# JiangongChen/ORB_SLAM3-1

Measured on AMD Instinct MI355X. Metric: tracking frames/s (ORB extract+match), higher is better.
Workload: dtype u8; 1 GPU; ORBextractor 640x480, 8 levels, 1000 features (configs[1]) + SearchByBoW 1000x1000 per frame (configs[2]); batch_per_gpu=256

## Files before the change

include/orbslam3_hip.h:

```cpp
#ifndef ORBSLAM3_HIP_H
#define ORBSLAM3_HIP_H

#include <stddef.h>
#include <stdint.h>

#ifdef __cplusplus
extern "C" {
#endif

#define ORBX_OK 0
#define ORBX_ERR_EMPTY (-1)
#define ORBX_ERR_CAPACITY (-2)
#define ORBX_ERR_ARG (-3)
#define ORBX_ERR_NO_DEVICE (-4)
#define ORBX_ERR_HIP (-5)
#define ORBX_ERR_INTERNAL (-6)

const char* orbx_last_error(void);
int orbx_device_count(void);


typedef struct OrbxKeyPoint {
    float x, y;
    float size;
// ... 36 lines not shown
                        const OrbxKeyPoint* kps_r, const uint8_t* desc_r, int n_r, float mb, float mbf, float* u_right, float* depth);
int orbx_stereo_matches_device(orbx_extractor* left, orbx_extractor* right, int batch,
                               const OrbxKeyPoint* d_kps_l, const uint8_t* d_desc_l, const int32_t* d_n_l,
                               const OrbxKeyPoint* d_kps_r, const uint8_t* d_desc_r, const int32_t* d_n_r, int cap,
                               float mb, float mbf, float* d_u_right, float* d_depth, void* stream);

int orbx_profile_enable(orbx_extractor* h, int on);
int orbx_profile_read(orbx_extractor* h, float* stage_ms, int n_stages);

int orbx_debug_blurred_level(orbx_extractor* h, int frame, int level, uint8_t* dst, int dst_stride);
int orbx_debug_candidates(orbx_extractor* h, int frame, int level, OrbxKeyPoint* out, int cap, int* n);
int orbx_debug_level_keypoints(orbx_extractor* h, int frame, int level, OrbxKeyPoint* out, int cap, int* n);
int orbx_debug_set_fast_corner_cap(orbx_extractor* h, int cap);
int orbx_debug_set_tail_delay(orbx_extractor* h, int microseconds);
int orbx_debug_last_schedule(orbx_extractor* h);
int orbx_debug_octree_waves(orbx_extractor* h, int launch);
int orbx_debug_octree_table(orbx_extractor* h, int level, int* depth, int* n_ini, int16_t* bounds, int cap);
int orbx_debug_resize_bands(orbx_extractor* h);
int orbx_debug_resize_rows(int src_h, int dst_h, uint32_t* rows, int* band_rows);
int orbx_debug_fast_scores(const uint8_t* patches, int n, int pitch, int* out);
int orbx_debug_orient_desc(orbx_extractor* h, int width, int height, int batch, const uint8_t* raw, const uint8_t* blurred, int pad_byte,
                           const int32_t* counts, const int32_t* keys, int cap, int guard_rows,
                           OrbxKeyPoint* kps, uint8_t* desc, OrbxKeyPoint* lvl_kps, int lvl_cap, int32_t* sel_caps);


int orbm_hamming(const uint8_t a[32], const uint8_t b[32]);

typedef struct OrbmFeatVec {
    int32_t n_nodes;
    const uint32_t* node_id;
// ... 514 lines not shown
```

orb_slam3-1_amd/capi.py:

```python
import ctypes as C
import os

import numpy as np

_PKG_DIR = os.path.dirname(os.path.abspath(__file__))
_LIB_PATH = os.path.join(_PKG_DIR, "liborbslam3_hip.so")

KP_DTYPE = np.dtype([("x", "f4"), ("y", "f4"), ("size", "f4"), ("angle", "f4"), ("response", "f4"),
                     ("octave", "i4"), ("class_id", "i4")])
assert KP_DTYPE.itemsize == 28

ORBX_OK, ORBX_ERR_EMPTY, ORBX_ERR_CAPACITY, ORBX_ERR_ARG, ORBX_ERR_NO_DEVICE, ORBX_ERR_HIP, ORBX_ERR_INTERNAL = 0, -1, -2, -3, -4, -5, -6


class OrbxError(RuntimeError):
    def __init__(self, code, msg):
        super().__init__("orbslam3_hip error %d: %s" % (code, msg))
        self.code = code


class FeatVec(C.Structure):
    _fields_ = [("n_nodes", C.c_int32), ("node_id", C.c_void_p), ("offset", C.c_void_p), ("feat", C.c_void_p)]


# ... 44 lines not shown
                                          C.c_void_p, C.c_void_p, C.c_int, C.c_void_p, C.c_void_p, C.c_void_p, C.c_void_p]
lib.orbx_max_keypoints.argtypes = [C.c_void_p]
lib.orbx_max_keypoints_for.argtypes = [C.c_void_p, C.c_int, C.c_int]
lib.orbx_levels.argtypes = [C.c_void_p]
lib.orbx_scale_factor.argtypes = [C.c_void_p]
lib.orbx_scale_factor.restype = C.c_float
lib.orbx_scale_tables.argtypes = [C.c_void_p] + [C.c_void_p] * 4
lib.orbx_features_per_level.argtypes = [C.c_void_p, C.c_void_p]
lib.orbx_pyramid_level_size.argtypes = [C.c_void_p, C.c_int, C.POINTER(C.c_int), C.POINTER(C.c_int)]
lib.orbx_pyramid_level.argtypes = [C.c_void_p, C.c_int, C.c_int, C.c_int, C.c_void_p, C.c_int]
lib.orbx_debug_blurred_level.argtypes = [C.c_void_p, C.c_int, C.c_int, C.c_void_p, C.c_int]
lib.orbx_debug_candidates.argtypes = [C.c_void_p, C.c_int, C.c_int, C.c_void_p, C.c_int, C.POINTER(C.c_int)]
lib.orbx_debug_level_keypoints.argtypes = [C.c_void_p, C.c_int, C.c_int, C.c_void_p, C.c_int, C.POINTER(C.c_int)]
lib.orbx_debug_set_tail_delay.argtypes = [C.c_void_p, C.c_int]
lib.orbx_debug_last_schedule.argtypes = [C.c_void_p]
lib.orbx_debug_octree_waves.argtypes = [C.c_void_p, C.c_int]
lib.orbx_debug_octree_table.argtypes = [C.c_void_p, C.c_int, C.POINTER(C.c_int), C.POINTER(C.c_int), C.c_void_p, C.c_int]
lib.orbx_debug_resize_bands.argtypes = [C.c_void_p]
lib.orbx_debug_resize_rows.argtypes = [C.c_int, C.c_int, C.c_void_p, C.POINTER(C.c_int)]
lib.orbx_debug_introsort.argtypes = [C.c_void_p, C.c_void_p, C.c_void_p, C.c_int]
lib.orbx_debug_wave_sort.argtypes = [C.c_void_p, C.c_void_p, C.c_void_p, C.c_int]
lib.orbx_debug_fast_scores.argtypes = [C.c_void_p, C.c_int, C.c_int, C.c_void_p]
lib.orbx_debug_orient_desc.argtypes = [C.c_void_p, C.c_int, C.c_int, C.c_int, C.c_void_p, C.c_void_p, C.c_int, C.c_void_p, C.c_void_p,
                                       C.c_int, C.c_int, C.c_void_p, C.c_void_p, C.c_void_p, C.c_int, C.c_void_p]
lib.orbx_debug_fast_atan2.restype = C.c_float
lib.orbx_debug_fast_atan2.argtypes = [C.c_float, C.c_float]
lib.orbx_debug_sincos.argtypes = [C.c_float, C.POINTER(C.c_float), C.POINTER(C.c_float)]


def _p(a):
# ... 138 lines not shown
        _check(lib.orbx_debug_blurred_level(self._h, frame, level, _p(out), out.strides[0]))
        return out

    def debug_set_fast_corner_cap(self, cap):
        lib.orbx_debug_set_fast_corner_cap.argtypes = [C.c_void_p, C.c_int]
        _check(lib.orbx_debug_set_fast_corner_cap(self._h, int(cap)))

    def debug_set_tail_delay(self, microseconds):
        _check(lib.orbx_debug_set_tail_delay(self._h, int(microseconds)))

    def debug_resize_bands(self):
        return bool(lib.orbx_debug_resize_bands(self._h))

    def debug_last_schedule(self):
        return int(lib.orbx_debug_last_schedule(self._h))

    def debug_octree_waves(self, launch):
        return int(lib.orbx_debug_octree_waves(self._h, launch))

    def debug_octree_table(self, level):
        depth, n_ini = C.c_int(), C.c_int()
        out = np.zeros(2 * 65537, np.int16)
        n = _check(lib.orbx_debug_octree_table(self._h, level, C.byref(depth), C.byref(n_ini), _p(out), out.size))
        nb = (1 << depth.value) + 1
        assert n == (n_ini.value + 1) * nb or n == 0
        return depth.value, n_ini.value, out[:n_ini.value * nb].reshape(n_ini.value, nb).copy(), out[n_ini.value * nb:n].copy()

    def candidates(self, level, frame=0, cap=200000):
        out = np.zeros(cap, KP_DTYPE)
        n = C.c_int()
# ... 2259 lines not shown
```

orb_slam3-1_amd/csrc/orbx_extractor.hip:

```cpp
#include <hip/hip_runtime.h>

#include <algorithm>
#include <cmath>
#include <cstdarg>
#include <cstdio>
#include <cstdlib>
#include <cstring>
#include <string>
#include <vector>

#include "hip_check.h"
#include "orbx_kernels.hip"

namespace orbx {

thread_local std::string g_last_error;

int fail(int code, const char* fmt, ...)
{
    char buf[512];
    va_list ap;
    va_start(ap, fmt);
    vsnprintf(buf, sizeof(buf), fmt, ap);
    va_end(ap);
// ... 65 lines not shown
        if (count <= n) return ORBX_OK;
        if (p) { (void)hipFree(p); p = nullptr; n = 0; }
        ORBX_HIP(hipMalloc((void**)&p, count * sizeof(T)));
        n = count;
        return ORBX_OK;
    }
    int upload(const std::vector<T>& v)
    {
        int r = ensure(v.size() ? v.size() : 1);
        if (r) return r;
        if (!v.empty()) ORBX_HIP(hipMemcpy(p, v.data(), v.size() * sizeof(T), hipMemcpyHostToDevice));
        return ORBX_OK;
    }
    void release() { if (p) (void)hipFree(p); p = nullptr; n = 0; }
};

}

using namespace orbx;

struct orbx_extractor {
    int device = 0;
    int nfeatures = 0, nlevels = 0, ini_th = 0, min_th = 0;
    float scale_factor_f = 0;
    double scale_factor_d = 0;
    std::vector<float> scale, inv_scale, sigma2, inv_sigma2;
    std::vector<int> nfeat;
    int taps[7];
    int max_kp = 0;

// ... 65 lines not shown
    int oct_split = 0, oct_pool_hi = 0;
    size_t oct_lds_hi = 0;
    int split_parts = 1;
    bool serial_schedule = false;
    bool last_resize_bands = false;
    int resize_band_min = 64;
    int resize_tail_first = 4;
    bool oct_dyn_off = false;
    int oct_dyn_max_batch = 64;
    int oct_waves_env = 0;
    int oct_waves_beside[3] = {2, 2, 2};
    int oct_small_max_waves = 32;
    int last_oct_waves[3] = {0, 0, 0};
    int oct_dyn_keys_beside = 6144;
    bool resize_beside = true;
    std::vector<hipStream_t> aux_streams;
    hipEvent_t ev_parts_fork = nullptr;
    std::vector<hipEvent_t> ev_parts_join;

    int setup_geometry(int w, int h);
    int ensure_batch(int batch);
    int enqueue(const uint8_t* d_imgs, bool level0_ready, int batch, int row_stride, size_t frame_stride,
                int lap0, int lap1, OrbxKeyPoint* o_kps, uint8_t* o_desc, int cap, int* o_n, int* o_mono, int* o_status,
                hipStream_t st);
    int launch_orient_desc(int f0, int n_frames, hipStream_t s, OrbxKeyPoint* o_kps, uint8_t* o_desc, int cap);
};

static void build_tables(orbx_extractor* e)
{
    const int nl = e->nlevels;
// ... 116 lines not shown
            while (c1 < (int)cells.size() && cells[c1].y0 == cells[c0].y0) c1++;
            const int n_row = c1 - c0;
            const int w_cell = std::max(cells[c0].x1 - cells[c0].x0 - 6, 1);
            static const int strip_width = getenv("ORBX_STRIP_WIDTH") ? std::max(48, std::min(atoi(getenv("ORBX_STRIP_WIDTH")), 250)) : kStripWidth;
            const int per = std::max(1, std::min(kStripMaxCells, (strip_width - 6) / w_cell));
            const int n_strips_row = (n_row + per - 1) / per;
            for (int k = 0; k < n_strips_row; k++) {
                const int a = c0 + (int)((long long)n_row * k / n_strips_row), b = c0 + (int)((long long)n_row * (k + 1) / n_strips_row);
                StripDesc sd;
                sd.level = (int16_t)l; sd.cell0 = (int16_t)a; sd.ncell = (int16_t)(b - a);
                sd.x0 = cells[a].x0; sd.x1 = cells[b - 1].x1; sd.y0 = cells[a].y0; sd.y1 = cells[a].y1; sd.pad = 0;
                strips.push_back(sd);
            }
            c0 = c1;
        }
        for (int y0 = 0; y0 < L.h; y0 += kBlurTH)
            for (int x0 = 0; x0 < L.w; x0 += kBlurTW) {
                TileDesc t; t.level = (int16_t)l; t.x0 = (int16_t)x0; t.y0 = (int16_t)y0;
                t.edge = (int16_t)((x0 == 0 ? 1 : 0) | (L.w <= x0 + kBlurTW + 2 ? 2 : 0));
                tiles.push_back(t);
            }
        if (l > 0) {
            const LevelDesc& P = levels[l - 1];
            const double scale_x = 1. / ((double)L.w / P.w);
            const int wpad = round_up(L.w, 4);
            std::vector<int> xofs(wpad, 0), yofs;
            std::vector<short> ia((size_t)wpad * 2, 0), ib;
            auto sat = sat_short;
            bool sums_ok = true;
            for (int dx = 0; dx < L.w; dx++) {
                float fx = (float)((dx + 0.5) * scale_x - 0.5);
                int sx = cv_floor_host(fx);
                fx -= sx;
                if (sx < 0) { fx = 0; sx = 0; }
                if (sx >= P.w - 1) { fx = 0; sx = P.w - 1; }
                xofs[dx] = sx;
// ... 161 lines not shown
        oct_dyn_keys = (int)std::min<size_t>((size_t)max_cand_cap, (150 * 1024 - node_bytes) / 8);
        if (const char* envd = getenv("ORBX_OCT_DYN_KEYS")) oct_dyn_keys = std::max(64, std::min(oct_dyn_keys, atoi(envd)));
        oct_dyn_lds = node_bytes + 8 * (size_t)oct_dyn_keys + 16;
    }
    if (!oct_nodes_hbm) {
        ORBX_HIP(hipFuncSetAttribute((const void*)k_octree<false>, hipFuncAttributeMaxDynamicSharedMemorySize, (int)node_bytes + 64));
        ORBX_HIP(hipFuncSetAttribute((const void*)k_octree<true>, hipFuncAttributeMaxDynamicSharedMemorySize, (int)std::max(oct_lds, oct_small_lds)));
        if (oct_dyn_keys > 0) ORBX_HIP(hipFuncSetAttribute((const void*)k_octree_dyn, hipFuncAttributeMaxDynamicSharedMemorySize, (int)oct_dyn_lds));
    } else {
        oct_lds = 64; oct_small_lds = 64;
    }
    ORBX_HIP(hipFuncSetAttribute((const void*)k_fast_strips, hipFuncAttributeMaxDynamicSharedMemorySize, (int)fast_lds));
    int r;
    if ((r = d_oct_tabs.upload(oct_tabs)) || (r = d_oct_bounds.upload(oct_bounds)) || (r = d_oct_maps.upload(oct_maps))) return r;
    if ((r = d_levels.upload(levels)) || (r = d_cells.upload(cells)) || (r = d_tiles.upload(tiles)) || (r = d_strips.upload(strip_recs))) return r;
    geo_w = w; geo_h = h;
    batch_cap = 0;
    return ORBX_OK;
}

int orbx_extractor::ensure_batch(int batch)
{
    if (batch <= batch_cap) return ORBX_OK;
    int r;
    const size_t B = (size_t)batch;
    if ((r = d_pyr.ensure(B * pyr_frame_bytes + 64)) || (r = d_blur.ensure(B * pyr_frame_bytes + 64)) ||
        (r = d_cand.ensure(B * cand_frame_entries)) || (r = d_scratch.ensure(B * 2 * cand_frame_entries)) ||
        (r = d_sel.ensure(B * sel_frame_entries)) || (r = d_cell_count.ensure(B * std::max<size_t>(cells.size(), 1))) ||
        (r = d_sel_count.ensure(B * nlevels)) || (r = d_kp_dst.ensure(B * sel_frame_entries)) ||
        (r = d_lvl_kps.ensure(B * sel_frame_entries)) || (r = d_n.ensure(B)) || (r = d_mono.ensure(B)) || (r = d_status.ensure(B)))
// ... 32 lines not shown
    hipLaunchKernelGGL(k_orient_desc, dim3((unsigned)(((long long)quads * n_frames + 7) / 8 * 8)), dim3(256), 0, s,
                       d_pyr.p + (size_t)f0 * pyr_frame_bytes, d_blur.p + (size_t)f0 * pyr_frame_bytes, pyr_frame_bytes,
                       d_levels.p, nlevels, d_sel.p + (size_t)f0 * sel_frame_entries, sel_frame_entries, d_sel_count.p + (size_t)f0 * nlevels,
                       d_kp_dst.p + (size_t)f0 * sel_frame_entries, sel_frame_entries,
                       o_kps + (size_t)f0 * cap, o_desc + (size_t)f0 * cap * 32, cap, d_lvl_kps.p + (size_t)f0 * sel_frame_entries, quads, n_frames);
    const hipError_t le = hipGetLastError();
    if (le != hipSuccess) return fail(ORBX_ERR_HIP, "launch of k_orient_desc: %s", hipGetErrorString(le));
    return ORBX_OK;
}

int orbx_extractor::enqueue(const uint8_t* d_imgs, bool level0_ready, int batch, int row_stride, size_t frame_stride,
                            int lap0, int lap1, OrbxKeyPoint* o_kps, uint8_t* o_desc, int cap, int* o_n, int* o_mono, int* o_status,
                            hipStream_t st)
{
    const int B = batch;
    ORBX_HIP(hipMemsetAsync(o_status, 0, sizeof(int) * B, st));
    int mark_i = 0;
    auto mark = [&]() { if (profile && mark_i < kProfEvents) (void)hipEventRecord(prof_ev[mark_i++], st); };
#define ORBX_LAUNCHED(name) do { const hipError_t le_ = hipGetLastError(); if (le_ != hipSuccess) return fail(ORBX_ERR_HIP, "launch of %s: %s", name, hipGetErrorString(le_)); } while (0)
    const bool in_place = !level0_ready && ((uintptr_t)d_imgs % 16 == 0) && (row_stride % 16 == 0) && (frame_stride % 16 == 0) && row_stride < (1 << 23);
    const int n_cells = (int)cells.size();

    auto run_range = [&](int f0, int nB, hipStream_t s, hipStream_t blur_s, bool marks) -> int {
        uint8_t* pyr = d_pyr.p + (size_t)f0 * pyr_frame_bytes;
        uint8_t* blr = d_blur.p + (size_t)f0 * pyr_frame_bytes;
        SrcImage lvl0;
        lvl0.base = nullptr; lvl0.frame_stride = 0; lvl0.stride = 0; lvl0.w = levels[0].w; lvl0.h = levels[0].h;
        if (in_place) { lvl0.base = d_imgs + (size_t)f0 * frame_stride; lvl0.frame_stride = frame_stride; lvl0.stride = row_stride; }
        if (marks) mark();
        if (!level0_ready && !in_place) {
            const LevelDesc& L0 = levels[0];
            dim3 g((L0.w / 4 + 255) / 256, L0.h, nB);
            hipLaunchKernelGGL(k_copy_level0, g, dim3(256), 0, s, d_imgs + (size_t)f0 * frame_stride, row_stride, frame_stride, pyr, pyr_frame_bytes, L0);
            ORBX_LAUNCHED("k_copy_level0");
        }
        if (marks) mark();
        int l_tail = (nB >= 64 && resize_tail_first >= 2 && resize_tail_first < nlevels) ? resize_tail_first : nlevels;
        for (int l = l_tail; l < nlevels; l++) if (resize_generic[l]) l_tail = nlevels;
        const bool chain_beside = resize_beside && blur_s && oct_stream && n_cells > 0 && l_tail < nlevels && l_tail > 1 &&
                                  !strips.empty() && strips[0].level == 0;
        hipStream_t rs = chain_beside ? oct_stream : s;
        if (chain_beside) { ORBX_HIP(hipEventRecord(ev_fork, s)); ORBX_HIP(hipStreamWaitEvent(rs, ev_fork, 0)); }
        bool resize_bands = false;
        for (int l = 1; l < l_tail; l++) {
            const LevelDesc& D = levels[l];
            const LevelDesc& P = levels[l - 1];
            SrcImage src;
            src.base = pyr + P.off; src.frame_stride = pyr_frame_bytes; src.stride = P.stride; src.w = P.w; src.h = P.h;
            if (l == 1 && in_place) src = lvl0;
            if (resize_generic[l]) {
                hipLaunchKernelGGL(k_resize_generic, dim3((D.w + 255) / 256, D.h, nB), dim3(256), 0, rs, src, pyr, pyr_frame_bytes, D,
                                   d_xofs[l].p, d_ialpha[l].p, d_yofs[l].p, d_ibeta[l].p);
                ORBX_LAUNCHED("k_resize_generic");
                continue;
            }
            if (nB < resize_band_min) {
                dim3 g(xcd_grid(((D.w + kResizeTileW - 1) / kResizeTileW) * ((D.h + kResizeRows - 1) / kResizeRows)), nB);
                hipLaunchKernelGGL(resize_sat[l] ? k_resize_tiles<true> : k_resize_tiles<false>, g, dim3(256), 0, rs, src, pyr, pyr_frame_bytes, D,
                                   d_qsx0[l].p, d_qsel[l].p, d_qalpha[l].p, d_rows[l].p);
                ORBX_LAUNCHED("k_resize_tiles");
                continue;
            }
            const int F = (nB >= 4 && resize_frames_fit(src.frame_stride) && resize_frames_fit(pyr_frame_bytes)) ? kResizeFrames : 1;
            dim3 g(xcd_grid(((D.w + resize_strip_w(F) - 1) / resize_strip_w(F)) * ((D.h + kResizeRows - 1) / kResizeRows)), (nB + F - 1) / F);
            auto kern = F == 1 ? (resize_sat[l] ? k_resize<1, true> : k_resize<1, false>) : (resize_sat[l] ? k_resize<kResizeFrames, true> : k_resize<kResizeFrames, false>);
            hipLaunchKernelGGL(kern, g, dim3(256), 0, rs, src, pyr, pyr_frame_bytes, D, nB, d_qsx0[l].p, d_qsel[l].p, d_qalpha[l].p, d_rows[l].p);
            resize_bands = true;
            ORBX_LAUNCHED("k_resize");
        }
        if (chain_beside) ORBX_HIP(hipEventRecord(ev_resize, rs));
        const bool small_batch = !oct_keys_forced && oct_small_keys > 0 && (long long)B * nlevels <= 512;
        const bool dyn_keys = !oct_keys_forced && !small_batch && oct_dyn_keys > 0 && B <= oct_dyn_max_batch && !oct_dyn_off;
        const int dyn_k = (blur_s && B >= 32) ? std::min(oct_dyn_keys, oct_dyn_keys_beside) : oct_dyn_keys;
        const size_t o_lds = small_batch ? oct_small_lds : (dyn_keys ? oct_dyn_lds - 8 * (size_t)(oct_dyn_keys - dyn_k) : oct_lds);
        const int o_keys = small_batch ? oct_small_keys : (dyn_keys ? dyn_k : oct_lds_keys);
        uint32_t* sel = d_sel.p + (size_t)f0 * sel_frame_entries;
        int* sel_cnt = d_sel_count.p + (size_t)f0 * nlevels;
        int* kp_dst = d_kp_dst.p + (size_t)f0 * sel_frame_entries;
        auto oct_kernel = oct_nodes_hbm ? k_octree<false, false> : (dyn_keys ? k_octree_dyn : (o_keys > 0 ? k_octree<true, true> : k_octree<false, true>));
        const bool two_launches = !oct_nodes_hbm && (o_keys == 0 || dyn_keys) && oct_split > 0 && oct_stream && blur_s;
        const int lv_lo = two_launches ? oct_split : nlevels;
        const bool oct_beside = B > 64;
        last_oct_waves[0] = last_oct_waves[1] = last_oct_waves[2] = 0;
        auto launch_octree = [&](hipStream_t qs, int lv0, int lv1, size_t lds, int pool, int keys, int which) {
            const int W = oct_waves_env ? oct_waves_env : (oct_beside ? oct_waves_beside[which] : 4);
            if (lv1 > lv0) last_oct_waves[which] = W;
            if (lv1 > lv0)
                hipLaunchKernelGGL(oct_kernel, dim3(lv1 - lv0, nB), dim3(64 * W), lds, qs, d_levels.p, d_cells.p, d_cand.p + (size_t)f0 * cand_frame_entries, (size_t)cand_frame_entries,
                                   d_cell_count.p + (size_t)f0 * std::max<size_t>(cells.size(), 1), n_cells, d_scratch.p + (size_t)f0 * 2 * cand_frame_entries, (size_t)2 * cand_frame_entries, pool, keys,
                                   sel, sel_frame_entries, sel_cnt, nlevels, o_status + f0,
                                   d_oct_nodes.p ? d_oct_nodes.p + (size_t)f0 * nlevels * oct_node_stride : nullptr, oct_node_stride, lv0, W > 1 ? oct_small_max_waves : 32,
                                   d_oct_tabs.p, d_oct_maps.p, d_oct_prefix.p + (size_t)f0 * oct_prefix_frame, oct_prefix_frame);
        };
        auto launch_blur = [&](hipStream_t bs) {
            hipLaunchKernelGGL(k_blur, dim3(xcd_grid((int)tiles.size()), nB), dim3(256), 0, bs, lvl0, pyr, in_place ? pyr : nullptr, blr, pyr_frame_bytes,
                               d_levels.p, d_tiles.p, (int)tiles.size(), taps[0], taps[1], taps[2], taps[3]);
        };
        bool oct0_early = false;
        bool tail_beside = false;
        uint32_t* cand = d_cand.p + (size_t)f0 * cand_frame_entries;
        int* cell_cnt = d_cell_count.p + (size_t)f0 * std::max<size_t>(cells.size(), 1);
        auto launch_fast = [&](hipStream_t fs, int s0, int s1) {
            if (s1 > s0)
                hipLaunchKernelGGL(k_fast_strips, dim3(xcd_grid(s1 - s0), nB), dim3(256), fast_lds, fs, lvl0, pyr, pyr_frame_bytes,
                                   d_strips.p + s0, s1 - s0, n_cells, ini_th, min_th, fast_layout, cand, (size_t)cand_frame_entries, cell_cnt);
        };
        int tail_strip = (int)strips.size();
        for (int si = (int)strips.size() - 1; si >= 0 && strips[si].level >= l_tail; si--) tail_strip = si;
        if (l_tail < nlevels) {
            ResizeTables T;
            std::memset(&T, 0, sizeof(T));
            for (int l = l_tail; l < nlevels; l++) { T.q_sx0[l] = d_qsx0[l].p; T.q_sel[l] = d_qsel[l].p; T.q_alpha[l] = d_qalpha[l].p; T.rows[l] = d_rows[l].p; }
            const bool beside = blur_s && oct_stream && n_cells > 0 && tail_strip > 0;
            hipStream_t ts = beside ? oct_stream : s;
            if (beside && !chain_beside) { ORBX_HIP(hipEventRecord(ev_fork, s)); ORBX_HIP(hipStreamWaitEvent(ts, ev_fork, 0)); }
            if (dbg_tail_delay_us > 0) hipLaunchKernelGGL(k_debug_spin, dim3(1), dim3(64), 0, ts, (long long)dbg_tail_delay_us * 100);
            bool tail_sat = false;
            for (int l = l_tail; l < nlevels; l++) tail_sat = tail_sat || resize_sat[l];
            hipLaunchKernelGGL(tail_sat ? k_resize_tail<true> : k_resize_tail<false>, dim3(nB), dim3(1024), 0, ts, pyr, pyr_frame_bytes, d_levels.p, T, l_tail, nlevels);
            ORBX_LAUNCHED("k_resize_tail");
            if (beside) {
                ORBX_HIP(hipEventRecord(ev_tail, ts));
                tail_beside = true;
                launch_fast(ts, tail_strip, (int)strips.size());
                ORBX_HIP(hipEventRecord(ev_oct_join, ts));
                int l1_strip = tail_strip;
                for (int si = tail_strip - 1; si >= 0 && strips[si].level >= 1; si--) l1_strip = si;
                if (two_launches && oct_split > 1 && l1_strip > 0 && l1_strip < tail_strip) {
                    launch_fast(s, 0, l1_strip);
                    ORBX_HIP(hipEventRecord(ev_fast0, s));
                    ORBX_HIP(hipStreamWaitEvent(blur_s, ev_fast0, 0));
                    launch_octree(blur_s, 0, 1, o_lds, oct_pool, o_keys, 0);
                    oct0_early = true;
                    if (chain_beside) ORBX_HIP(hipStreamWaitEvent(s, ev_resize, 0));
                    launch_fast(s, l1_strip, tail_strip);
                } else if (chain_beside && l1_strip > 0 && l1_strip < tail_strip) {
                    launch_fast(s, 0, l1_strip);
                    ORBX_HIP(hipStreamWaitEvent(s, ev_resize, 0));
                    launch_fast(s, l1_strip, tail_strip);
                } else {
                    if (chain_beside) ORBX_HIP(hipStreamWaitEvent(s, ev_resize, 0));
                    launch_fast(s, 0, tail_strip);
                }
                ORBX_HIP(hipStreamWaitEvent(blur_s, ev_oct_join, 0));
            } else {
                if (marks) mark();
                if (n_cells > 0) launch_fast(s, 0, (int)strips.size());
            }
        } else {
            if (marks) mark();
            if (n_cells > 0) launch_fast(s, 0, (int)strips.size());
        }
        ORBX_LAUNCHED("k_fast_strips");
        if (marks) mark();
        hipStream_t os = blur_s ? blur_s : s;
        if (blur_s) {
            ORBX_HIP(hipEventRecord(ev_fork, s));
            ORBX_HIP(hipStreamWaitEvent(blur_s, ev_fork, 0));
        }
        if (two_launches) {
            ORBX_HIP(hipStreamWaitEvent(oct_stream, ev_fork, 0));
            {
                const int k_hi = dyn_keys ? std::max(64, o_keys / 2) : 0;
                launch_octree(oct_stream, oct_split, nlevels, oct_lds_hi + 8 * (size_t)k_hi, oct_pool_hi, k_hi, 2);
            }
            ORBX_HIP(hipEventRecord(ev_oct_join, oct_stream));
        }
        launch_octree(os, oct0_early ? 1 : 0, lv_lo, o_lds, oct_pool, o_keys, 1);
        if (blur_s) {
            if (tail_beside) ORBX_HIP(hipStreamWaitEvent(s, ev_tail, 0));
            launch_blur(s);
        }
        last_octree_variant = (oct_nodes_hbm ? 0 : (dyn_keys ? 3 : (o_keys > 0 ? 1 : 2))) | (two_launches ? 4 : 0) | (oct0_early ? 8 : 0) | (in_place ? 16 : 0) | (tail_beside ? 32 : 0) | (chain_beside ? 64 : 0);
        last_resize_bands = resize_bands;
        if (two_launches) ORBX_HIP(hipStreamWaitEvent(os, ev_oct_join, 0));
        ORBX_LAUNCHED("k_octree / k_blur");
        if (marks) mark();
        hipLaunchKernelGGL(k_index, dim3(nB), dim3(64), 0, os, d_levels.p, nlevels, sel, sel_frame_entries, sel_cnt,
                           lap0, lap1, cap, kp_dst, sel_frame_entries, o_n + f0, o_mono + f0, o_status + f0);
        ORBX_LAUNCHED("k_index");
        if (marks) mark();
        if (blur_s) { ORBX_HIP(hipEventRecord(ev_join, blur_s)); ORBX_HIP(hipStreamWaitEvent(s, ev_join, 0)); }
        else launch_blur(s);
        if (marks) mark();
        if (const int lr = launch_orient_desc(f0, nB, s, o_kps, o_desc, cap)) return lr;
        if (marks) mark();
        return ORBX_OK;
    };

    int parts = 1;
    if (!profile && split_parts > 1 && B >= 32 * split_parts) parts = std::min(split_parts, 1 + (int)aux_streams.size());
    int r;
    if (parts == 1) {
        if ((r = run_range(0, B, st, (!profile && !serial_schedule && side_stream && B >= 32) ? side_stream : nullptr, true))) return r;
    } else {
        ORBX_HIP(hipEventRecord(ev_parts_fork, st));
        for (int p = 0; p < parts; p++) {
            const int f0 = (int)((long long)B * p / parts), f1 = (int)((long long)B * (p + 1) / parts);
            hipStream_t s = p == 0 ? st : aux_streams[p - 1];
            if (p > 0) ORBX_HIP(hipStreamWaitEvent(s, ev_parts_fork, 0));
            if ((r = run_range(f0, f1 - f0, s, nullptr, false))) return r;
            if (p > 0) { ORBX_HIP(hipEventRecord(ev_parts_join[p - 1], s)); ORBX_HIP(hipStreamWaitEvent(st, ev_parts_join[p - 1], 0)); }
        }
    }
    prof_marks = mark_i;
    prof_stream = st;
    ORBX_HIP(hipGetLastError());
    last_batch = B;
    return ORBX_OK;
}

extern "C" {

int orbx_profile_enable(orbx_extractor* e, int on)
{
    if (!e) return fail(ORBX_ERR_ARG, "NULL handle");
    ORBX_HIP(hipSetDevice(e->device));
    if (on && !e->prof_ev[0])
        for (int i = 0; i < orbx_extractor::kProfEvents; i++) ORBX_HIP(hipEventCreate(&e->prof_ev[i]));
    e->profile = on != 0;
    e->prof_marks = 0;
    return ORBX_OK;
}
// ... 36 lines not shown
    if (hipStreamCreateWithFlags(&e->stream, hipStreamNonBlocking) != hipSuccess) { delete e; return fail(ORBX_ERR_HIP, "stream create failed"); }
    if (hipStreamCreateWithFlags(&e->side_stream, hipStreamNonBlocking) != hipSuccess ||
        hipEventCreateWithFlags(&e->ev_fork, hipEventDisableTiming) != hipSuccess ||
        hipEventCreateWithFlags(&e->ev_join, hipEventDisableTiming) != hipSuccess ||
        hipEventCreateWithFlags(&e->ev_parts_fork, hipEventDisableTiming) != hipSuccess ||
        hipStreamCreateWithFlags(&e->oct_stream, hipStreamNonBlocking) != hipSuccess ||
        hipEventCreateWithFlags(&e->ev_oct_join, hipEventDisableTiming) != hipSuccess ||
        hipEventCreateWithFlags(&e->ev_tail, hipEventDisableTiming) != hipSuccess ||
        hipEventCreateWithFlags(&e->ev_resize, hipEventDisableTiming) != hipSuccess ||
        hipEventCreateWithFlags(&e->ev_fast0, hipEventDisableTiming) != hipSuccess) { orbx_destroy(e); return fail(ORBX_ERR_HIP, "side stream create failed"); }
    if (const char* env = getenv("ORBX_SERIAL")) e->serial_schedule = atoi(env) != 0;
    if (const char* env = getenv("ORBX_SPLIT")) e->split_parts = std::max(1, std::min(atoi(env), 4));
    if (const char* env = getenv("ORBX_RESIZE_TAIL")) e->resize_tail_first = atoi(env);
    if (const char* env = getenv("ORBX_RESIZE_BAND_MIN")) e->resize_band_min = std::max(atoi(env), 1);
    if (const char* env = getenv("ORBX_RESIZE_BESIDE")) e->resize_beside = atoi(env) != 0;
    if (const char* env = getenv("ORBX_OCT_DYN")) e->oct_dyn_off = atoi(env) == 0;
    if (const char* env = getenv("ORBX_OCT_DYN_MAXB")) e->oct_dyn_max_batch = atoi(env);
    if (const char* env = getenv("ORBX_OCT_WAVES")) { const int wv = atoi(env); if (wv == 1 || wv == 2 || wv == 4) e->oct_waves_env = wv; }
    if (const char* env = getenv("ORBX_OCT_TAB_DEPTH")) e->oct_tab_depth_max = std::max(0, std::min(kOctTabMaxDepth, atoi(env)));
    if (const char* env = getenv("ORBX_OCT_SMALL_MAX")) e->oct_small_max_waves = std::max(0, std::min(64, atoi(env)));
    if (const char* env = getenv("ORBX_OCT_WAVES_BESIDE")) {
        for (int i = 0; i < 3 && env[i]; i++) { const int wv = env[i] - '0'; if (wv == 1 || wv == 2 || wv == 4) e->oct_waves_beside[i] = wv; }
    }
    if (const char* env = getenv("ORBX_OCT_DYN_KEYS_BESIDE")) e->oct_dyn_keys_beside = std::max(64, atoi(env));
    for (int i = 0; i + 1 < e->split_parts; i++) {
        hipStream_t s = nullptr; hipEvent_t ev = nullptr;
        if (hipStreamCreateWithFlags(&s, hipStreamNonBlocking) != hipSuccess || hipEventCreateWithFlags(&ev, hipEventDisableTiming) != hipSuccess) {
            if (s) (void)hipStreamDestroy(s);
            break;
        }
// ... 257 lines not shown
    OctTabDesc t;
    ORBX_HIP(hipMemcpy(&t, e->d_oct_tabs.p + level, sizeof(t), hipMemcpyDeviceToHost));
    const int n = t.n_ini > 0 ? (t.n_ini + 1) * ((1 << t.depth) + 1) : 0;
    if (n > cap) return fail(ORBX_ERR_CAPACITY, "%d boundaries, room for %d", n, cap);
    if (n > 0) ORBX_HIP(hipMemcpy(bounds, e->d_oct_bounds.p + t.bounds_off, sizeof(int16_t) * n, hipMemcpyDeviceToHost));
    *depth = t.depth; *n_ini = t.n_ini;
    return n;
}

int orbx_debug_last_schedule(orbx_extractor* e)
{
    if (!e) return fail(ORBX_ERR_ARG, "NULL handle");
    return e->last_octree_variant;
}

int orbx_debug_set_fast_corner_cap(orbx_extractor* e, int cap)
{
    if (!e) return fail(ORBX_ERR_ARG, "NULL handle");
    e->fast_corner_cap = cap > 0 ? std::min(cap, 4096) : 0;
    e->geo_w = e->geo_h = 0;
    return ORBX_OK;
}

int orbx_debug_introsort(int32_t* count, int32_t* ulx, int32_t* node, int n)
{
    if (n < 0) return ORBX_ERR_ARG;
    std::vector<SortNode> v(n);
    for (int i = 0; i < n; i++) { v[i].count = count[i]; v[i].ulx = ulx[i]; v[i].node = node[i]; }
    std::vector<int> stack(3 * kIntrosortStack);
    introsort_nodes(v.data(), n, stack.data());
// ... 222 lines not shown
```

orb_slam3-1_amd/csrc/orbx_fast_strips.inc:

```

struct StripDesc {
    int16_t level;
    int16_t cell0, ncell;
    int16_t x0, x1;
    int16_t y0, y1;
    int16_t pad;
};

constexpr int kStripMaxCells = 8;
constexpr int kStripMapPitchMax = 4 * 64 + 8;

struct __attribute__((aligned(16))) StripTab {
    int32_t cx0[kStripMaxCells];
    int32_t iw[kStripMaxCells];
    int32_t slot_off[kStripMaxCells], slot_cap[kStripMaxCells];
    uint8_t colcell[(kStripMapPitchMax + 15) & ~15];
};

struct __attribute__((aligned(16))) StripRec {
    uint32_t src_off;
    uint32_t stride;
    uint32_t y0_xa;
    uint32_t th_nch;
    uint32_t g0_qoff;
// ... 68 lines not shown
{
    __builtin_amdgcn_fence(__ATOMIC_RELEASE, "wavefront");
    __builtin_amdgcn_wave_barrier();
    __builtin_amdgcn_fence(__ATOMIC_ACQUIRE, "wavefront");
}

#ifdef ORBX_FAST_TIMING
__device__ unsigned long long d_fast_prof[16];
#define ORBX_FTICK(k) if (threadIdx.x == 0) { const long long t_now = clock64(); atomicAdd(&d_fast_prof[(k) + fallback_slot], (unsigned long long)(t_now - t_prev)); t_prev = t_now; }
#else
#define ORBX_FTICK(k)
#endif
__global__ __launch_bounds__(256) void k_fast_strips(SrcImage lvl0, const uint8_t* __restrict__ pyr, size_t frame_stride,
                                                     const StripRec* __restrict__ recs, int n_strips, int n_cells,
                                                     int ini_th, int min_th, FastLds Z,
                                                     uint32_t* __restrict__ cand, size_t cand_frame_stride, int* __restrict__ cell_count)
{
    extern __shared__ __align__(16) uint8_t smem[];
    __shared__ StripTab s_tab;
    __shared__ int s_total[kStripMaxCells];
    __shared__ int s_seg[4][kStripMaxCells + 1];
#ifdef ORBX_FAST_TIMING
    long long t_prev = clock64();
    int fallback_slot = 0;
#endif

    const int strip_idx = xcd_remap(blockIdx.x, gridDim.x, blockIdx.y);
    if (strip_idx >= n_strips) return;
    const StripRec* S = recs + strip_idx;
    const int frame = blockIdx.y;
    const int tid = threadIdx.x, lane = tid & 63, wave = __builtin_amdgcn_readfirstlane(tid >> 6);
    const uint4 h0 = ((const uint4*)S)[0], h1 = ((const uint4*)S)[1];
    uint4 tab_chunk = make_uint4(0u, 0u, 0u, 0u);
    if (wave == 0) tab_chunk = ((const uint4*)&S->tab)[min(lane, kStripTabChunks - 1)];
    const int sy0 = (int)(h0.z & 0xFFFFu), xa = (int)(h0.z >> 16);
    const int th = (int)(h0.w & 0xFFFFu), nch = (int)(h0.w >> 16), ih = th - 6;
    const int g0 = (int)(h1.x & 0xFFFFu), qoff = (int)(h1.x >> 16);
    const int ncell = (int)(h1.y & 0xFFFFu), cell0 = (int)(h1.y >> 16);
    const uint32_t inv_nch = h1.w;
#if defined(ORBX_FAST_CUT)
    if ((int)threadIdx.x < ncell) cell_count[(size_t)frame * n_cells + cell0 + threadIdx.x] = 0;
// ... 268 lines not shown
```

Baseline: 320,500 frames/s.

## Split blur across streams, bind event records to launches, fold status clear into FAST

The blur launch is split into two tile ranges. Tiles for the tail pyramid levels are blurred on the side stream right after the tail resize and FAST, so the main stream no longer waits on the tail event before blurring. Event records are attached to kernel launches through hipExtLaunchKernelGGL instead of separate hipEventRecord calls, and the status memset is folded into the first FAST kernel as a single-thread clear. Together these aim to cut cross-stream waits, launch count and API overhead, at the cost of more complex scheduling and new ordering assumptions about the tile list.

```diff
diff --git a/include/orbslam3_hip.h b/include/orbslam3_hip.h
--- a/include/orbslam3_hip.h
+++ b/include/orbslam3_hip.h
@@ -74,6 +74,8 @@
 int orbx_debug_set_fast_corner_cap(orbx_extractor* h, int cap);
 int orbx_debug_set_tail_delay(orbx_extractor* h, int microseconds);
 int orbx_debug_last_schedule(orbx_extractor* h);
+int orbx_debug_last_handoffs(orbx_extractor* h);
+int orbx_debug_blur_tile_split(float scale_factor, int nlevels, int width, int height, int level, int16_t* tile_levels, int cap, int* split);
 int orbx_debug_octree_waves(orbx_extractor* h, int launch);
 int orbx_debug_octree_table(orbx_extractor* h, int level, int* depth, int* n_ini, int16_t* bounds, int cap);
 int orbx_debug_resize_bands(orbx_extractor* h);
diff --git a/orb_slam3-1_amd/capi.py b/orb_slam3-1_amd/capi.py
--- a/orb_slam3-1_amd/capi.py
+++ b/orb_slam3-1_amd/capi.py
@@ -82,6 +82,8 @@
 lib.orbx_debug_level_keypoints.argtypes = [C.c_void_p, C.c_int, C.c_int, C.c_void_p, C.c_int, C.POINTER(C.c_int)]
 lib.orbx_debug_set_tail_delay.argtypes = [C.c_void_p, C.c_int]
 lib.orbx_debug_last_schedule.argtypes = [C.c_void_p]
+lib.orbx_debug_last_handoffs.argtypes = [C.c_void_p]
+lib.orbx_debug_blur_tile_split.argtypes = [C.c_float, C.c_int, C.c_int, C.c_int, C.c_int, C.c_void_p, C.c_int, C.POINTER(C.c_int)]
 lib.orbx_debug_octree_waves.argtypes = [C.c_void_p, C.c_int]
 lib.orbx_debug_octree_table.argtypes = [C.c_void_p, C.c_int, C.POINTER(C.c_int), C.POINTER(C.c_int), C.c_void_p, C.c_int]
 lib.orbx_debug_resize_bands.argtypes = [C.c_void_p]
@@ -250,6 +252,9 @@
 
     def debug_last_schedule(self):
         return int(lib.orbx_debug_last_schedule(self._h))
+
+    def debug_last_handoffs(self):
+        return int(lib.orbx_debug_last_handoffs(self._h))
 
     def debug_octree_waves(self, launch):
         return int(lib.orbx_debug_octree_waves(self._h, launch))
diff --git a/orb_slam3-1_amd/csrc/orbx_extractor.hip b/orb_slam3-1_amd/csrc/orbx_extractor.hip
--- a/orb_slam3-1_amd/csrc/orbx_extractor.hip
+++ b/orb_slam3-1_amd/csrc/orbx_extractor.hip
@@ -1,4 +1,5 @@
 #include <hip/hip_runtime.h>
+#include <hip/hip_ext.h>
 
 #include <algorithm>
 #include <cmath>
@@ -103,6 +104,25 @@
     }
     void release() { if (p) (void)hipFree(p); p = nullptr; n = 0; }
 };
+
+static void append_blur_tiles(int level, int w, int h, std::vector<TileDesc>& tiles)
+{
+    for (int y0 = 0; y0 < h; y0 += kBlurTH)
+        for (int x0 = 0; x0 < w; x0 += kBlurTW) {
+            TileDesc t; t.level = (int16_t)level; t.x0 = (int16_t)x0; t.y0 = (int16_t)y0;
+            t.edge = (int16_t)((x0 == 0 ? 1 : 0) | (w <= x0 + kBlurTW + 2 ? 2 : 0));
+            tiles.push_back(t);
+        }
+}
+
+static bool blur_tile_split(const std::vector<TileDesc>& tiles, int level, int* split)
+{
+    size_t t = 0;
+    while (t < tiles.size() && tiles[t].level < level) t++;
+    *split = (int)t;
+    for (; t < tiles.size(); t++) if (tiles[t].level < level) return false;
+    return true;
+}
 
 }
 
@@ -198,6 +218,11 @@
     int last_oct_waves[3] = {0, 0, 0};
     int oct_dyn_keys_beside = 6144;
     bool resize_beside = true;
+    bool blur_split = true;
+    bool bind_records = true;
+    bool status_in_fast = true;
+    int blur_split_tile = 0;
+    int last_handoffs = 0;
     std::vector<hipStream_t> aux_streams;
     hipEvent_t ev_parts_fork = nullptr;
     std::vector<hipEvent_t> ev_parts_join;
@@ -344,12 +369,7 @@
             }
             c0 = c1;
         }
-        for (int y0 = 0; y0 < L.h; y0 += kBlurTH)
-            for (int x0 = 0; x0 < L.w; x0 += kBlurTW) {
-                TileDesc t; t.level = (int16_t)l; t.x0 = (int16_t)x0; t.y0 = (int16_t)y0;
-                t.edge = (int16_t)((x0 == 0 ? 1 : 0) | (L.w <= x0 + kBlurTW + 2 ? 2 : 0));
-                tiles.push_back(t);
-            }
+        append_blur_tiles(l, L.w, L.h, tiles);
         if (l > 0) {
             const LevelDesc& P = levels[l - 1];
             const double scale_x = 1. / ((double)L.w / P.w);
@@ -541,6 +561,9 @@
     int r;
     if ((r = d_oct_tabs.upload(oct_tabs)) || (r = d_oct_bounds.upload(oct_bounds)) || (r = d_oct_maps.upload(oct_maps))) return r;
     if ((r = d_levels.upload(levels)) || (r = d_cells.upload(cells)) || (r = d_tiles.upload(tiles)) || (r = d_strips.upload(strip_recs))) return r;
+    blur_split_tile = (int)tiles.size();
+    if (resize_tail_first >= 2 && resize_tail_first < nlevels && !blur_tile_split(tiles, resize_tail_first, &blur_split_tile))
+        return fail(ORBX_ERR_INTERNAL, "the blur tiles of levels %d.. are not one range of the tile list", resize_tail_first);
     geo_w = w; geo_h = h;
     batch_cap = 0;
     return ORBX_OK;
@@ -603,12 +626,28 @@
                             hipStream_t st)
 {
     const int B = batch;
-    ORBX_HIP(hipMemsetAsync(o_status, 0, sizeof(int) * B, st));
     int mark_i = 0;
     auto mark = [&]() { if (profile && mark_i < kProfEvents) (void)hipEventRecord(prof_ev[mark_i++], st); };
 #define ORBX_LAUNCHED(name) do { const hipError_t le_ = hipGetLastError(); if (le_ != hipSuccess) return fail(ORBX_ERR_HIP, "launch of %s: %s", name, hipGetErrorString(le_)); } while (0)
     const bool in_place = !level0_ready && ((uintptr_t)d_imgs % 16 == 0) && (row_stride % 16 == 0) && (frame_stride % 16 == 0) && row_stride < (1 << 23);
     const int n_cells = (int)cells.size();
+    int parts = 1;
+    if (!profile && split_parts > 1 && B >= 32 * split_parts) parts = std::min(split_parts, 1 + (int)aux_streams.size());
+    hipStream_t side_q = (parts == 1 && !profile && !serial_schedule && side_stream && B >= 32) ? side_stream : nullptr;
+    auto tail_plan = [&](int nB, int& l_tail, int& tail_strip) {
+        l_tail = (nB >= 64 && resize_tail_first >= 2 && resize_tail_first < nlevels) ? resize_tail_first : nlevels;
+        for (int l = l_tail; l < nlevels; l++) if (resize_generic[l]) l_tail = nlevels;
+        tail_strip = (int)strips.size();
+        for (int si = (int)strips.size() - 1; si >= 0 && strips[si].level >= l_tail; si--) tail_strip = si;
+    };
+    bool status_by_fast = false;
+    if (status_in_fast && side_q && oct_stream && n_cells > 0 && (level0_ready || in_place)) {
+        int lt, ts;
+        tail_plan(B, lt, ts);
+        status_by_fast = lt < nlevels && ts > 0;
+    }
+    if (!status_by_fast) ORBX_HIP(hipMemsetAsync(o_status, 0, sizeof(int) * B, st));
+    int handoffs = status_by_fast ? 4 : 0;
 
     auto run_range = [&](int f0, int nB, hipStream_t s, hipStream_t blur_s, bool marks) -> int {
         uint8_t* pyr = d_pyr.p + (size_t)f0 * pyr_frame_bytes;
@@ -624,8 +663,17 @@
             ORBX_LAUNCHED("k_copy_level0");
         }
         if (marks) mark();
-        int l_tail = (nB >= 64 && resize_tail_first >= 2 && resize_tail_first < nlevels) ? resize_tail_first : nlevels;
-        for (int l = l_tail; l < nlevels; l++) if (resize_generic[l]) l_tail = nlevels;
+        int l_tail, tail_strip;
+        tail_plan(nB, l_tail, tail_strip);
+        auto launch_ev = [&](hipEvent_t ev, auto kern, dim3 grid, dim3 block, size_t lds, hipStream_t q, auto... args) -> hipError_t {
+            if (ev && bind_records) {
+                hipExtLaunchKernelGGL(kern, grid, block, (uint32_t)lds, q, nullptr, ev, 0, args...);
+                handoffs |= 2;
+                return hipSuccess;
+            }
+            hipLaunchKernelGGL(kern, grid, block, lds, q, args...);
+            return ev ? hipEventRecord(ev, q) : hipSuccess;
+        };
         const bool chain_beside = resize_beside && blur_s && oct_stream && n_cells > 0 && l_tail < nlevels && l_tail > 1 &&
                                   !strips.empty() && strips[0].level == 0;
         hipStream_t rs = chain_beside ? oct_stream : s;
@@ -637,27 +685,27 @@
             SrcImage src;
             src.base = pyr + P.off; src.frame_stride = pyr_frame_bytes; src.stride = P.stride; src.w = P.w; src.h = P.h;
             if (l == 1 && in_place) src = lvl0;
+            const hipEvent_t ev = (chain_beside && l == l_tail - 1) ? ev_resize : nullptr;
             if (resize_generic[l]) {
-                hipLaunchKernelGGL(k_resize_generic, dim3((D.w + 255) / 256, D.h, nB), dim3(256), 0, rs, src, pyr, pyr_frame_bytes, D,
-                                   d_xofs[l].p, d_ialpha[l].p, d_yofs[l].p, d_ibeta[l].p);
+                ORBX_HIP(launch_ev(ev, k_resize_generic, dim3((D.w + 255) / 256, D.h, nB), dim3(256), 0, rs, src, pyr, pyr_frame_bytes, D,
+                                   d_xofs[l].p, d_ialpha[l].p, d_yofs[l].p, d_ibeta[l].p));
                 ORBX_LAUNCHED("k_resize_generic");
                 continue;
             }
             if (nB < resize_band_min) {
                 dim3 g(xcd_grid(((D.w + kResizeTileW - 1) / kResizeTileW) * ((D.h + kResizeRows - 1) / kResizeRows)), nB);
-                hipLaunchKernelGGL(resize_sat[l] ? k_resize_tiles<true> : k_resize_tiles<false>, g, dim3(256), 0, rs, src, pyr, pyr_frame_bytes, D,
-                                   d_qsx0[l].p, d_qsel[l].p, d_qalpha[l].p, d_rows[l].p);
+                ORBX_HIP(launch_ev(ev, resize_sat[l] ? k_resize_tiles<true> : k_resize_tiles<false>, g, dim3(256), 0, rs, src, pyr, pyr_frame_bytes, D,
+                                   d_qsx0[l].p, d_qsel[l].p, d_qalpha[l].p, d_rows[l].p));
                 ORBX_LAUNCHED("k_resize_tiles");
                 continue;
             }
             const int F = (nB >= 4 && resize_frames_fit(src.frame_stride) && resize_frames_fit(pyr_frame_bytes)) ? kResizeFrames : 1;
             dim3 g(xcd_grid(((D.w + resize_strip_w(F) - 1) / resize_strip_w(F)) * ((D.h + kResizeRows - 1) / kResizeRows)), (nB + F - 1) / F);
             auto kern = F == 1 ? (resize_sat[l] ? k_resize<1, true> : k_resize<1, false>) : (resize_sat[l] ? k_resize<kResizeFrames, true> : k_resize<kResizeFrames, false>);
-            hipLaunchKernelGGL(kern, g, dim3(256), 0, rs, src, pyr, pyr_frame_bytes, D, nB, d_qsx0[l].p, d_qsel[l].p, d_qalpha[l].p, d_rows[l].p);
+            ORBX_HIP(launch_ev(ev, kern, g, dim3(256), 0, rs, src, pyr, pyr_frame_bytes, D, nB, d_qsx0[l].p, d_qsel[l].p, d_qalpha[l].p, d_rows[l].p));
             resize_bands = true;
             ORBX_LAUNCHED("k_resize");
         }
-        if (chain_beside) ORBX_HIP(hipEventRecord(ev_resize, rs));
         const bool small_batch = !oct_keys_forced && oct_small_keys > 0 && (long long)B * nlevels <= 512;
         const bool dyn_keys = !oct_keys_forced && !small_batch && oct_dyn_keys > 0 && B <= oct_dyn_max_batch && !oct_dyn_off;
         const int dyn_k = (blur_s && B >= 32) ? std::min(oct_dyn_keys, oct_dyn_keys_beside) : oct_dyn_keys;
@@ -671,117 +719,124 @@
         const int lv_lo = two_launches ? oct_split : nlevels;
         const bool oct_beside = B > 64;
         last_oct_waves[0] = last_oct_waves[1] = last_oct_waves[2] = 0;
-        auto launch_octree = [&](hipStream_t qs, int lv0, int lv1, size_t lds, int pool, int keys, int which) {
+        auto launch_octree = [&](hipStream_t qs, int lv0, int lv1, size_t lds, int pool, int keys, int which, hipEvent_t ev) -> hipError_t {
             const int W = oct_waves_env ? oct_waves_env : (oct_beside ? oct_waves_beside[which] : 4);
-            if (lv1 > lv0) last_oct_waves[which] = W;
-            if (lv1 > lv0)
-                hipLaunchKernelGGL(oct_kernel, dim3(lv1 - lv0, nB), dim3(64 * W), lds, qs, d_levels.p, d_cells.p, d_cand.p + (size_t)f0 * cand_frame_entries, (size_t)cand_frame_entries,
-                                   d_cell_count.p + (size_t)f0 * std::max<size_t>(cells.size(), 1), n_cells, d_scratch.p + (size_t)f0 * 2 * cand_frame_entries, (size_t)2 * cand_frame_entries, pool, keys,
-                                   sel, sel_frame_entries, sel_cnt, nlevels, o_status + f0,
-                                   d_oct_nodes.p ? d_oct_nodes.p + (size_t)f0 * nlevels * oct_node_stride : nullptr, oct_node_stride, lv0, W > 1 ? oct_small_max_waves : 32,
-                                   d_oct_tabs.p, d_oct_maps.p, d_oct_prefix.p + (size_t)f0 * oct_prefix_frame, oct_prefix_frame);
+            if (lv1 <= lv0) return ev ? hipEventRecord(ev, qs) : hipSuccess;
+            last_oct_waves[which] = W;
+            return launch_ev(ev, oct_kernel, dim3(lv1 - lv0, nB), dim3(64 * W), lds, qs, d_levels.p, d_cells.p, d_cand.p + (size_t)f0 * cand_frame_entries, (size_t)cand_frame_entries,
+                             d_cell_count.p + (size_t)f0 * std::max<size_t>(cells.size(), 1), n_cells, d_scratch.p + (size_t)f0 * 2 * cand_frame_entries, (size_t)2 * cand_frame_entries, pool, keys,
+                             sel, sel_frame_entries, sel_cnt, nlevels, o_status + f0,
+                             d_oct_nodes.p ? d_oct_nodes.p + (size_t)f0 * nlevels * oct_node_stride : nullptr, oct_node_stride, lv0, W > 1 ? oct_small_max_waves : 32,
+                             d_oct_tabs.p, d_oct_maps.p, d_oct_prefix.p + (size_t)f0 * oct_prefix_frame, oct_prefix_frame);
         };
-        auto launch_blur = [&](hipStream_t bs) {
-            hipLaunchKernelGGL(k_blur, dim3(xcd_grid((int)tiles.size()), nB), dim3(256), 0, bs, lvl0, pyr, in_place ? pyr : nullptr, blr, pyr_frame_bytes,
-                               d_levels.p, d_tiles.p, (int)tiles.size(), taps[0], taps[1], taps[2], taps[3]);
+        auto launch_blur = [&](hipStream_t bs, int t0, int t1, hipEvent_t ev) -> hipError_t {
+            if (t1 <= t0) return ev ? hipEventRecord(ev, bs) : hipSuccess;
+            return launch_ev(ev, k_blur, dim3(xcd_grid(t1 - t0), nB), dim3(256), 0, bs, lvl0, pyr, (in_place && t0 == 0) ? pyr : nullptr, blr, pyr_frame_bytes,
+                             d_levels.p, d_tiles.p + t0, t1 - t0, taps[0], taps[1], taps[2], taps[3]);
         };
+        const int n_tiles = (int)tiles.size();
         bool oct0_early = false;
         bool tail_beside = false;
         uint32_t* cand = d_cand.p + (size_t)f0 * cand_frame_entries;
         int* cell_cnt = d_cell_count.p + (size_t)f0 * std::max<size_t>(cells.size(), 1);
-        auto launch_fast = [&](hipStream_t fs, int s0, int s1) {
-            if (s1 > s0)
-                hipLaunchKernelGGL(k_fast_strips, dim3(xcd_grid(s1 - s0), nB), dim3(256), fast_lds, fs, lvl0, pyr, pyr_frame_bytes,
-                                   d_strips.p + s0, s1 - s0, n_cells, ini_th, min_th, fast_layout, cand, (size_t)cand_frame_entries, cell_cnt);
+        bool clear_pending = status_by_fast;
+        auto launch_fast = [&](hipStream_t fs, int s0, int s1, hipEvent_t ev) -> hipError_t {
+            if (s1 <= s0) return ev ? hipEventRecord(ev, fs) : hipSuccess;
+            int* clear = (clear_pending && fs == s) ? o_status + f0 : nullptr;
+            if (clear) clear_pending = false;
+            return launch_ev(ev, k_fast_strips, dim3(xcd_grid(s1 - s0), nB), dim3(256), fast_lds, fs, lvl0, pyr, pyr_frame_bytes,
+                             d_strips.p + s0, s1 - s0, n_cells, ini_th, min_th, fast_layout, cand, (size_t)cand_frame_entries, cell_cnt, clear);
         };
-        int tail_strip = (int)strips.size();
-        for (int si = (int)strips.size() - 1; si >= 0 && strips[si].level >= l_tail; si--) tail_strip = si;
+        const bool beside = l_tail < nlevels && blur_s && oct_stream && n_cells > 0 && tail_strip > 0;
+        const bool blur_ranges = blur_split && beside && l_tail == resize_tail_first && blur_split_tile > 0 && blur_split_tile < n_tiles;
+        bool fork_recorded = false;
         if (l_tail < nlevels) {
             ResizeTables T;
             std::memset(&T, 0, sizeof(T));
             for (int l = l_tail; l < nlevels; l++) { T.q_sx0[l] = d_qsx0[l].p; T.q_sel[l] = d_qsel[l].p; T.q_alpha[l] = d_qalpha[l].p; T.rows[l] = d_rows[l].p; }
-            const bool beside = blur_s && oct_stream && n_cells > 0 && tail_strip > 0;
             hipStream_t ts = beside ? oct_stream : s;
             if (beside && !chain_beside) { ORBX_HIP(hipEventRecord(ev_fork, s)); ORBX_HIP(hipStreamWaitEvent(ts, ev_fork, 0)); }
             if (dbg_tail_delay_us > 0) hipLaunchKernelGGL(k_debug_spin, dim3(1), dim3(64), 0, ts, (long long)dbg_tail_delay_us * 100);
             bool tail_sat = false;
             for (int l = l_tail; l < nlevels; l++) tail_sat = tail_sat || resize_sat[l];
-            hipLaunchKernelGGL(tail_sat ? k_resize_tail<true> : k_resize_tail<false>, dim3(nB), dim3(1024), 0, ts, pyr, pyr_frame_bytes, d_levels.p, T, l_tail, nlevels);
+            ORBX_HIP(launch_ev((beside && !blur_ranges) ? ev_tail : nullptr, tail_sat ? k_resize_tail<true> : k_resize_tail<false>, dim3(nB), dim3(1024), 0, ts,
+                               pyr, pyr_frame_bytes, d_levels.p, T, l_tail, nlevels));
             ORBX_LAUNCHED("k_resize_tail");
             if (beside) {
-                ORBX_HIP(hipEventRecord(ev_tail, ts));
                 tail_beside = true;
-                launch_fast(ts, tail_strip, (int)strips.size());
-                ORBX_HIP(hipEventRecord(ev_oct_join, ts));
+                ORBX_HIP(launch_fast(ts, tail_strip, (int)strips.size(), blur_ranges ? nullptr : ev_oct_join));
+                if (blur_ranges) ORBX_HIP(launch_blur(ts, blur_split_tile, n_tiles, ev_oct_join));
                 int l1_strip = tail_strip;
                 for (int si = tail_strip - 1; si >= 0 && strips[si].level >= 1; si--) l1_strip = si;
                 if (two_launches && oct_split > 1 && l1_strip > 0 && l1_strip < tail_strip) {
-                    launch_fast(s, 0, l1_strip);
-                    ORBX_HIP(hipEventRecord(ev_fast0, s));
+                    ORBX_HIP(launch_fast(s, 0, l1_strip, ev_fast0));
                     ORBX_HIP(hipStreamWaitEvent(blur_s, ev_fast0, 0));
-                    launch_octree(blur_s, 0, 1, o_lds, oct_pool, o_keys, 0);
+                    ORBX_HIP(launch_octree(blur_s, 0, 1, o_lds, oct_pool, o_keys, 0, nullptr));
                     oct0_early = true;
                     if (chain_beside) ORBX_HIP(hipStreamWaitEvent(s, ev_resize, 0));
-                    launch_fast(s, l1_strip, tail_strip);
+                    ORBX_HIP(launch_fast(s, l1_strip, tail_strip, ev_fork));
                 } else if (chain_beside && l1_strip > 0 && l1_strip < tail_strip) {
-                    launch_fast(s, 0, l1_strip);
+                    ORBX_HIP(launch_fast(s, 0, l1_strip, nullptr));
                     ORBX_HIP(hipStreamWaitEvent(s, ev_resize, 0));
-                    launch_fast(s, l1_strip, tail_strip);
+                    ORBX_HIP(launch_fast(s, l1_strip, tail_strip, ev_fork));
                 } else {
                     if (chain_beside) ORBX_HIP(hipStreamWaitEvent(s, ev_resize, 0));
-                    launch_fast(s, 0, tail_strip);
+                    ORBX_HIP(launch_fast(s, 0, tail_strip, ev_fork));
                 }
+                fork_recorded = true;
                 ORBX_HIP(hipStreamWaitEvent(blur_s, ev_oct_join, 0));
             } else {
                 if (marks) mark();
-                if (n_cells > 0) launch_fast(s, 0, (int)strips.size());
+                if (n_cells > 0) ORBX_HIP(launch_fast(s, 0, (int)strips.size(), nullptr));
             }
         } else {
             if (marks) mark();
-            if (n_cells > 0) launch_fast(s, 0, (int)strips.size());
+            if (n_cells > 0) ORBX_HIP(launch_fast(s, 0, (int)strips.size(), nullptr));
         }
         ORBX_LAUNCHED("k_fast_strips");
+        if (clear_pending) return fail(ORBX_ERR_INTERNAL, "no FAST launch on the launch stream took the status clear");
         if (marks) mark();
         hipStream_t os = blur_s ? blur_s : s;
         if (blur_s) {
-            ORBX_HIP(hipEventRecord(ev_fork, s));
+            if (!fork_recorded) ORBX_HIP(hipEventRecord(ev_fork, s));
             ORBX_HIP(hipStreamWaitEvent(blur_s, ev_fork, 0));
         }
         if (two_launches) {
             ORBX_HIP(hipStreamWaitEvent(oct_stream, ev_fork, 0));
             {
                 const int k_hi = dyn_keys ? std::max(64, o_keys / 2) : 0;
-                launch_octree(oct_stream, oct_split, nlevels, oct_lds_hi + 8 * (size_t)k_hi, oct_pool_hi, k_hi, 2);
+                ORBX_HIP(launch_octree(oct_stream, oct_split, nlevels, oct_lds_hi + 8 * (size_t)k_hi, oct_pool_hi, k_hi, 2, ev_oct_join));
             }
-            ORBX_HIP(hipEventRecord(ev_oct_join, oct_stream));
-        }
-        launch_octree(os, oct0_early ? 1 : 0, lv_lo, o_lds, oct_pool, o_keys, 1);
+        }
+        ORBX_HIP(launch_octree(os, oct0_early ? 1 : 0, lv_lo, o_lds, oct_pool, o_keys, 1, nullptr));
         if (blur_s) {
-            if (tail_beside) ORBX_HIP(hipStreamWaitEvent(s, ev_tail, 0));
-            launch_blur(s);
-        }
+            if (blur_ranges) ORBX_HIP(launch_blur(s, 0, blur_split_tile, nullptr));
+            else {
+                if (tail_beside) ORBX_HIP(hipStreamWaitEvent(s, ev_tail, 0));
+                ORBX_HIP(launch_blur(s, 0, n_tiles, nullptr));
+            }
+        }
+        if (blur_ranges) handoffs |= 1;
         last_octree_variant = (oct_nodes_hbm ? 0 : (dyn_keys ? 3 : (o_keys > 0 ? 1 : 2))) | (two_launches ? 4 : 0) | (oct0_early ? 8 : 0) | (in_place ? 16 : 0) | (tail_beside ? 32 : 0) | (chain_beside ? 64 : 0);
         last_resize_bands = resize_bands;
         if (two_launches) ORBX_HIP(hipStreamWaitEvent(os, ev_oct_join, 0));
         ORBX_LAUNCHED("k_octree / k_blur");
         if (marks) mark();
-        hipLaunchKernelGGL(k_index, dim3(nB), dim3(64), 0, os, d_levels.p, nlevels, sel, sel_frame_entries, sel_cnt,
-                           lap0, lap1, cap, kp_dst, sel_frame_entries, o_n + f0, o_mono + f0, o_status + f0);
+        ORBX_HIP(launch_ev(blur_s ? ev_join : nullptr, k_index, dim3(nB), dim3(64), 0, os, d_levels.p, nlevels, sel, sel_frame_entries, sel_cnt,
+                           lap0, lap1, cap, kp_dst, sel_frame_entries, o_n + f0, o_mono + f0, o_status + f0));
         ORBX_LAUNCHED("k_index");
         if (marks) mark();
-        if (blur_s) { ORBX_HIP(hipEventRecord(ev_join, blur_s)); ORBX_HIP(hipStreamWaitEvent(s, ev_join, 0)); }
-        else launch_blur(s);
+        if (blur_s) ORBX_HIP(hipStreamWaitEvent(s, ev_join, 0));
+        else ORBX_HIP(launch_blur(s, 0, n_tiles, nullptr));
         if (marks) mark();
         if (const int lr = launch_orient_desc(f0, nB, s, o_kps, o_desc, cap)) return lr;
         if (marks) mark();
         return ORBX_OK;
     };
 
-    int parts = 1;
-    if (!profile && split_parts > 1 && B >= 32 * split_parts) parts = std::min(split_parts, 1 + (int)aux_streams.size());
     int r;
     if (parts == 1) {
-        if ((r = run_range(0, B, st, (!profile && !serial_schedule && side_stream && B >= 32) ? side_stream : nullptr, true))) return r;
+        if ((r = run_range(0, B, st, side_q, true))) return r;
     } else {
         ORBX_HIP(hipEventRecord(ev_parts_fork, st));
         for (int p = 0; p < parts; p++) {
@@ -796,6 +851,7 @@
     prof_stream = st;
     ORBX_HIP(hipGetLastError());
     last_batch = B;
+    last_handoffs = handoffs;
     return ORBX_OK;
 }
 
@@ -862,6 +918,9 @@
     if (const char* env = getenv("ORBX_RESIZE_TAIL")) e->resize_tail_first = atoi(env);
     if (const char* env = getenv("ORBX_RESIZE_BAND_MIN")) e->resize_band_min = std::max(atoi(env), 1);
     if (const char* env = getenv("ORBX_RESIZE_BESIDE")) e->resize_beside = atoi(env) != 0;
+    if (const char* env = getenv("ORBX_BLUR_SPLIT")) e->blur_split = atoi(env) != 0;
+    if (const char* env = getenv("ORBX_BIND_RECORDS")) e->bind_records = atoi(env) != 0;
+    if (const char* env = getenv("ORBX_STATUS_IN_FAST")) e->status_in_fast = atoi(env) != 0;
     if (const char* env = getenv("ORBX_OCT_DYN")) e->oct_dyn_off = atoi(env) == 0;
     if (const char* env = getenv("ORBX_OCT_DYN_MAXB")) e->oct_dyn_max_batch = atoi(env);
     if (const char* env = getenv("ORBX_OCT_WAVES")) { const int wv = atoi(env); if (wv == 1 || wv == 2 || wv == 4) e->oct_waves_env = wv; }
@@ -1149,6 +1208,28 @@
     return e->last_octree_variant;
 }
 
+int orbx_debug_last_handoffs(orbx_extractor* e)
+{
+    if (!e) return fail(ORBX_ERR_ARG, "NULL handle");
+    return e->last_handoffs;
+}
+
+int orbx_debug_blur_tile_split(float scale_factor, int nlevels, int width, int height, int level, int16_t* tile_levels, int cap, int* split)
+{
+    if (!tile_levels || !split || nlevels < 1 || nlevels > kMaxLevels || !(scale_factor > 1.0f) || width < 1 || height < 1)
+        return fail(ORBX_ERR_ARG, "bad tile split request");
+    orbx_extractor e;
+    e.nfeatures = 1; e.nlevels = nlevels; e.scale_factor_f = scale_factor; e.scale_factor_d = (double)scale_factor;
+    build_tables(&e);
+    std::vector<TileDesc> tiles;
+    for (int l = 0; l < nlevels; l++)
+        append_blur_tiles(l, (int)std::nearbyintf((float)width * e.inv_scale[l]), (int)std::nearbyintf((float)height * e.inv_scale[l]), tiles);
+    if ((int)tiles.size() > cap) return fail(ORBX_ERR_CAPACITY, "%d tiles, room for %d", (int)tiles.size(), cap);
+    for (size_t t = 0; t < tiles.size(); t++) tile_levels[t] = tiles[t].level;
+    if (!blur_tile_split(tiles, level, split)) return fail(ORBX_ERR_INTERNAL, "the blur tiles of levels %d.. are not one range of the tile list", level);
+    return (int)tiles.size();
+}
+
 int orbx_debug_set_fast_corner_cap(orbx_extractor* e, int cap)
 {
     if (!e) return fail(ORBX_ERR_ARG, "NULL handle");
diff --git a/orb_slam3-1_amd/csrc/orbx_fast_strips.inc b/orb_slam3-1_amd/csrc/orbx_fast_strips.inc
--- a/orb_slam3-1_amd/csrc/orbx_fast_strips.inc
+++ b/orb_slam3-1_amd/csrc/orbx_fast_strips.inc
@@ -106,7 +106,8 @@
 __global__ __launch_bounds__(256) void k_fast_strips(SrcImage lvl0, const uint8_t* __restrict__ pyr, size_t frame_stride,
                                                      const StripRec* __restrict__ recs, int n_strips, int n_cells,
                                                      int ini_th, int min_th, FastLds Z,
-                                                     uint32_t* __restrict__ cand, size_t cand_frame_stride, int* __restrict__ cell_count)
+                                                     uint32_t* __restrict__ cand, size_t cand_frame_stride, int* __restrict__ cell_count,
+                                                     int* __restrict__ status_clear)
 {
     extern __shared__ __align__(16) uint8_t smem[];
     __shared__ StripTab s_tab;
@@ -117,6 +118,7 @@
     int fallback_slot = 0;
 #endif
 
+    if (status_clear != nullptr && blockIdx.x == 0 && threadIdx.x == 0) status_clear[blockIdx.y] = 0;
     const int strip_idx = xcd_remap(blockIdx.x, gridDim.x, blockIdx.y);
     if (strip_idx >= n_strips) return;
     const StripRec* S = recs + strip_idx;
```

New measurement: 329,900 frames/s (median of 6 runs). 3.0% higher.
